# aniketntnu/WordDiffusion

Measured on AMD Instinct MI355X. Metric: denoised 64x256 word images/sec (1000-step DDPM), whole job, higher is better.
Workload: dtype bf16x3; 1 GPU; BASELINE configs[1]: batch 64 per GPU of 64x256 crops = [64,4,8,32] latents, 1000-step DDPM (999 executed steps), base unet.py UNetModel (320 ch, mult (1,1), 4 heads, 339 writers), random-init synthetic weights; variant=base, batch_per_gpu=64, noise_steps=1000, executed_steps_per_image=999, precision=split-bf16 MFMA x3, fp32 accumulate (<=1e-4 of the fp32 reference), output_finite=True

## Files before the change

### worddiffusion_amd/csrc/wd_gemm.hip

```cpp
#include <stdlib.h>

#include "wd_common.h"
#include "wd_gemm_epi.h"
#include "wd_gemm_priv.h"


namespace {

constexpr int BK = 32;

__device__ __forceinline__ int lds_off(int row, int ch) { return row * 64 + ((ch ^ ((row >> 2) & 3)) << 4); }
__device__ __forceinline__ int lds_off16(int row, int ch) { return row * 64 + ((ch ^ ((0 - (row >> 2)) & 3)) << 4); }


template <int BM, int BN, int TN, int NT>
__device__ __forceinline__ void wd_epilogue_lds(const wd_gemm_args& a, const f32x16 (&acc)[TN], char* smem, const int m0,
                                                const int n0, const int wm, const int wn, const int wcols, const int kh,
                                                const int nkh, const int tid, const int sidx = 0) {
    constexpr int LDE = BN + 4;
    float* ep = reinterpret_cast<float*>(smem);
    const int lane = tid & 63;
    const int frow = lane & 31, fhalf = lane >> 5;
    asm volatile("s_waitcnt vmcnt(0)" ::: "memory");
    __syncthreads();
// ... 2060 lines not shown
        if (!wd_epilogue_vec_ok(a)) return WD_EINVAL;
        if (a.tile == 0) a.tile = bm * 1000 + bn;
    }
    if (a.ksplit > 1 && (!a.ws || a.act == WD_ACT_GEGLU || a.w_layout == 1)) return WD_EINVAL;
    if (a.ln_gamma) {
        if (a.w_layout != 3 || (a.tile && a.tile != 64320) || a.n != 320 || a.ksplit > 1 || !a.ln_beta || !a.out_hi || (a.out_pl_ld & 3) ||
            ((reinterpret_cast<uintptr_t>(a.ln_gamma) | reinterpret_cast<uintptr_t>(a.ln_beta)) & 15) ||
            ((reinterpret_cast<uintptr_t>(a.out_hi) | reinterpret_cast<uintptr_t>(a.out_lo)) & 7) || a.act == WD_ACT_GEGLU)
            return WD_EINVAL;
        a.tile = 64320;
        a.ksplit = 1;
    }
    if (a.gn_gamma) {
        if (!a.gn_beta || !a.stat_part || !a.out_hi || (!a.ws && a.tile != 64080) || a.hw_out != 64 || a.m % 64 || a.n % 160 || a.gn_cpg <= 0 ||
            40 % a.gn_cpg || a.stat_cpg <= 0 || a.gn_cpg % a.stat_cpg || a.act != WD_ACT_NONE || a.resid_rows || a.w_layout == 1)
            return WD_EINVAL;
        if (!wd_epilogue_vec_ok(a) ||
            ((reinterpret_cast<uintptr_t>(a.ws) | reinterpret_cast<uintptr_t>(a.gn_gamma) | reinterpret_cast<uintptr_t>(a.gn_beta)) & 15))
            return WD_EINVAL;
        a.tickets = nullptr;
    }
    if (a.w_layout == 1) {
        a.ksplit = 1;
        a.tickets = nullptr;
    }
    if (a.nsrc < 1 || a.nsrc > 2 || (a.npass != 1 && a.npass != 3)) return WD_EINVAL;
    if (a.m <= 0 || a.n <= 0 || a.hw_out <= 0 || !a.w_hi || (a.npass == 3 && !a.w_lo)) return WD_EINVAL;
    if (!a.out_f32 && !a.out_hi) return WD_EINVAL;
    long k = 0;
    for (int s = 0; s < a.nsrc; ++s) {
        const wd_src& q = a.src[s];
        if (s == 0 && a.a32) {
            if (a.w_layout != 3 || a.npass != 3 || (a.tile && a.tile != 64320) || a.n % 320 || a.hw_out % 64 || !a.a32_part || !a.a32_gamma ||
                !a.a32_beta || a.a32_nchunk <= 0 || a.a32_pcpg <= 0 || a.a32_cpg <= 0 || a.a32_cpg % a.a32_pcpg || q.c % a.a32_cpg ||
                q.c > 1024 || a.a32_ld < q.c || (a.a32_ld & 3) || (reinterpret_cast<uintptr_t>(a.a32) & 15) || q.hw_src <= 0)
                return WD_EINVAL;
        } else if (!q.hi || (a.npass == 3 && !q.lo)) return WD_EINVAL;
        if (q.c <= 0 || q.c % BK || q.ld % 8 || q.ntaps < 1) return WD_EINVAL;
        if (!q.gather && q.ntaps != 1) return WD_EINVAL;
        if (q.gather && q.hw_src <= 0) return WD_EINVAL;
        k += (long)q.ntaps * q.c;
    }
    if (k != a.ktot) return WD_EINVAL;
    {
        const long lim = 0x7FFFFFF0L;
        if ((long)a.n * a.ktot * 2 >= lim) return WD_EINVAL;
        for (int s = 0; s < a.nsrc; ++s) {
            const wd_src& q = a.src[s];
            const long rows = q.gather ? (long)((a.m + a.hw_out - 1) / a.hw_out) * q.hw_src : (long)a.m;
            if ((s == 0 && a.a32) ? rows * a.a32_ld * 4 >= lim : rows * q.ld * 2 >= lim) return WD_EINVAL;
        }
    }
    if (a.act == WD_ACT_GEGLU && (a.n % 64 || a.tile == 0)) return WD_EINVAL;
    if (a.rowvec && a.rowvec_ld <= 0) return WD_EINVAL;
    if (a.resid && a.resid_ld <= 0) return WD_EINVAL;
    {
        const int nout = a.act == WD_ACT_GEGLU ? a.n / 2 : a.n;
        if ((a.out_f32 && a.out_ld < nout) || (a.out_hi && a.out_pl_ld < nout) || (a.resid && a.resid_ld < nout) ||
            (a.rowvec && a.rowvec_ld < nout))
            return WD_EINVAL;
        for (int s = 0; s < a.nsrc; ++s)
            if (!(s == 0 && a.a32) && a.src[s].ld < a.src[s].c) return WD_EINVAL;
    }

    if (a.w_layout == 3) {
        bool ok = a.src[0].ntaps <= 9 && (a.nsrc == 1 || (a.src[1].gather == nullptr && a.src[1].ntaps == 1));
        for (int s = 0; s < a.nsrc; ++s) ok = ok && (a.src[s].c % 64 == 0);
        if (!ok) return WD_EINVAL;
        const wd_src& q0 = a.src[0];
        const bool same3 = q0.ntaps == 9 && q0.gather && a.slab_rows > 0 && q0.hw_src == a.hw_out && a.hw_out % a.slab_rows == 0;
        const bool down3 = a.tile == 64080 && q0.ntaps == 9 && q0.gather && a.slab_rows > 0 && q0.hw_src == 4 * a.hw_out;
        if (!same3 && !down3) a.slab_rows = 0;
        a.tickets = nullptr;
        if (a.tile == 64080) {
            if (!wd_gemmq_applies(a)) return WD_EINVAL;
            if (a.gn_gamma && (40 % a.gn_cpg || 80 % a.gn_cpg)) return WD_EINVAL;
            r.a = a, r.kernel = K_GEMMQ;
            return WD_OK;
        }
        const int nk64 = a.ktot / 64;
        if (a.ksplit == 0) a.ksplit = a.ws ? wd_auto_ksplit(a.tile, a.m, a.n, nk64, a.ws_floats) : 1;
        if (a.ksplit > 1 && (nk64 < a.ksplit || (long)a.ksplit * a.m * a.n > a.ws_floats)) a.ksplit = 1;
        if (a.gn_gamma && a.ksplit <= 1) return WD_EINVAL;
        r.a = a, r.kernel = K_GEMMW;
        return WD_OK;
    }
#ifndef WDIFF_EXPERIMENTAL
    if (a.w_layout == 1) return WD_EINVAL;
#else
    if (a.w_layout == 1) {
        if (a.src[0].ntaps > 9 || a.slab_rows <= 0) return WD_EINVAL;
        if (a.nsrc == 2 && (a.src[1].gather || a.src[1].ntaps != 1)) return WD_EINVAL;
        if (a.tile == 0) a.tile = (a.act == WD_ACT_GEGLU || a.n % 160) ? 128064 : 128160;
        if (a.act == WD_ACT_GEGLU && a.n % (a.tile % 1000)) return WD_EINVAL;
        if (a.slab_rows > 192) return WD_EINVAL;
        if (a.tile != 128064 && a.tile != 128128 && a.tile != 128160) return WD_EINVAL;
        r.a = a, r.kernel = K_SLAB;
        return WD_OK;
    }
#endif
    bool conv3 = false;
    if (a.w_layout == 2) {
        const wd_src& q0 = a.src[0];
        static const int conv3_mode = getenv("WDIFF_CONV3") ? atoi(getenv("WDIFF_CONV3")) : 0;
#ifdef WDIFF_EXPERIMENTAL
        const bool conv3_env = conv3_mode != 0 || (a.dbg & 0x1000);
#else
        const bool conv3_env = false;
        (void)conv3_mode;
#endif
        const bool same3 = q0.ntaps == 9 && q0.gather && a.slab_rows > 0 && q0.hw_src == a.hw_out && a.hw_out % a.slab_rows == 0;
        conv3 = conv3_env && same3 && q0.c % 64 == 0 && a.act != WD_ACT_GEGLU && (a.tile == 0 || a.tile == 128160) &&
                (a.nsrc == 1 || (!a.src[1].gather && a.src[1].ntaps == 1 && a.src[1].c % 64 == 0));
        if (conv3) a.tile = 128160;
        a.w_layout = 0;
        static const bool arith_env = getenv("WDIFF_GEMM_ARITH_TAB") ? atoi(getenv("WDIFF_GEMM_ARITH_TAB")) != 0 : true;
        if (!same3 || !arith_env) a.slab_rows = 0;
    } else if (a.w_layout == 0) {
        a.slab_rows = 0;
    } else if (a.w_layout != 0) {
        return WD_EINVAL;
    }
    bool v2ok = (a.ktot % BK2 == 0) && !getenv("WDIFF_GEMM_V1");
    for (int s = 0; s < a.nsrc; ++s) v2ok = v2ok && (a.src[s].c % BK2 == 0);
    v2ok = v2ok && a.src[0].ntaps <= 9 && (a.nsrc == 1 || (a.src[1].gather == nullptr && a.src[1].ntaps == 1));
    const int nk64 = a.ktot / BK2;
    int tile = a.tile;
    if (tile == 0)
        tile = wd_auto_tile(a.m, a.n, nk64, v2ok && a.ws && a.ksplit == 0 && a.act != WD_ACT_GEGLU, a.ws_floats);
    if (a.ksplit == 0) {
        a.ksplit = (v2ok && a.ws && a.act != WD_ACT_GEGLU) ? wd_auto_ksplit(tile, a.m, a.n, nk64, a.ws_floats) : 1;
    }
    if (a.act == WD_ACT_GEGLU && a.n % (tile % 1000)) return WD_EINVAL;
    if (a.ksplit > 1 && (!v2ok || nk64 < a.ksplit || (long)a.ksplit * a.m * a.n > a.ws_floats)) a.ksplit = 1;
    bool use_v4 = false;
    if (tile == 128160) {
        static const int v4_env = getenv("WDIFF_GEMM_V4") ? atoi(getenv("WDIFF_GEMM_V4")) : 2;
        const long wgs = (long)((a.m + 127) / 128) * ((a.n + 159) / 160) * a.ksplit;
        use_v4 = v2ok && !a.stat_part && (v4_env == 1 || (v4_env == 2 && wgs >= 512) || (a.dbg & 0x400));
    }
    {
        static const bool fuse_env = getenv("WDIFF_GEMM_FUSE_COMBINE") ? atoi(getenv("WDIFF_GEMM_FUSE_COMBINE")) != 0 : false;
        const int bn = tile % 1000, bm = tile / 1000;
        const long ntile = (long)((a.m + bm - 1) / bm) * ((a.n + bn - 1) / bn);
        const bool aligned = (a.n & 3) == 0 && a.n % bn == 0 && wd_epilogue_vec_ok(a) && (reinterpret_cast<uintptr_t>(a.ws) & 15) == 0;
        if (!((fuse_env || (a.dbg & 0x2000)) && a.tickets && a.ksplit > 1 && v2ok && !use_v4 && !conv3 && aligned && ntile <= a.ntickets))
            a.tickets = nullptr;
    }
    if (a.gn_gamma && !(a.ksplit > 1 && tile == 128160 && v2ok && !use_v4 && !conv3)) return WD_EINVAL;
    static const int stagger_min = getenv("WDIFF_GEMM_STAGGER_MIN") ? atoi(getenv("WDIFF_GEMM_STAGGER_MIN")) : 10;
    static const bool stagger = getenv("WDIFF_GEMM_STAGGER") ? atoi(getenv("WDIFF_GEMM_STAGGER")) != 0 : true;
    static const bool m16 = getenv("WDIFF_GEMM_M16") ? atoi(getenv("WDIFF_GEMM_M16")) != 0 : true;
    static const bool pp = getenv("WDIFF_GEMM_PP") ? atoi(getenv("WDIFF_GEMM_PP")) != 0 : false;
    a.tile = tile;
#ifdef WDIFF_EXPERIMENTAL
    if (conv3 && v2ok) return r.a = a, r.kernel = K_CONV3, WD_OK;
#endif
    if (tile != 128064 && tile != 128160 && tile != 128128 && tile != 64064) return WD_EINVAL;
    if (tile == 128160) {
        if (use_v4) return r.a = a, r.kernel = K_V4, WD_OK;
#ifdef WDIFF_EXPERIMENTAL
        static const int v8_env = getenv("WDIFF_GEMM_V8") ? atoi(getenv("WDIFF_GEMM_V8")) : 0;
        bool v8ok = a.ktot % 32 == 0 && a.src[0].ntaps <= 9 && !a.stat_part && !a.gn_gamma && a.act != WD_ACT_GEGLU &&
                    (a.nsrc == 1 || (a.src[1].gather == nullptr && a.src[1].ntaps == 1));
        for (int s8 = 0; s8 < a.nsrc; ++s8) v8ok = v8ok && (a.src[s8].c % 32 == 0);
        if (v8ok && (v8_env == 1 || (a.dbg & 0x80000))) {
// ... 98 lines not shown
```

### worddiffusion_amd/csrc/wd_gemm_priv.h

```cpp
#pragma once
#include "wd_common.h"

int wd_gemmw_launch(const wd_gemm_args& a, hipStream_t st);
int wd_gemm_launch_reduce(const wd_gemm_args& a, hipStream_t st, int bm);
bool wd_gemmq_applies(const wd_gemm_args& a);
int wd_gemmq_launch(const wd_gemm_args& a, hipStream_t st);
```

### worddiffusion_amd/csrc/wd_gemmw.hip

```cpp
#include "wd_gemm_epi.h"
#include "wd_gemm_priv.h"

namespace {

constexpr int WNT = 512;

typedef __attribute__((ext_vector_type(4))) unsigned w_u32x4;

__device__ __forceinline__ int w_lds_off(int row, int ch) { return row * 128 + ((ch ^ ((row >> 1) & 7)) << 4); }

template <int NPASS, int RH, bool A32>
__global__ void __launch_bounds__(WNT, 1) wd_gemmw_kernel(const wd_gemm_args a, const int nbn, const int nbm) {
#if defined(__HIP_DEVICE_COMPILE__)
    constexpr int NPL = (NPASS == 1) ? 1 : 2;
    constexpr int BM = 64 * RH, BN = 320 / RH;
    constexpr int A_PL = BM * 128;
    constexpr int STAGE = NPL * A_PL;
    constexpr uint32_t WD_OOB = 0x80000000u;

    extern __shared__ __attribute__((aligned(16))) char smem[];
    int* s_tab = reinterpret_cast<int*>(smem + 2 * STAGE);

    const int ntile = nbn * nbm;
    const int nwg = ntile * a.ksplit;
    int wg;
    {
        const int bid = blockIdx.x;
        const int q = nwg >> 3, r = nwg & 7, xcd = bid & 7, loc = bid >> 3;
        wg = (xcd < r ? xcd * (q + 1) : r * (q + 1) + (xcd - r) * q) + loc;
    }
    const int sidx = wg % a.ksplit;
    wg /= a.ksplit;
    const int bn_i = wg % nbn, bm_i = wg / nbn;
    const int m0 = bm_i * BM, n0 = bn_i * BN;

    const int tid = threadIdx.x;
    const int lane = tid & 63;
    const int wave = __builtin_amdgcn_readfirstlane(tid >> 6);
    const int kh = wave >> 2;
    const int rh = RH == 2 ? (wave >> 1) & 1 : 0;
    const int cg = RH == 2 ? wave & 1 : wave & 3;
    const int l15 = lane & 15, lq = lane >> 4;

    {
        const int nt0 = a.src[0].ntaps;
        const int32_t* g0 = a.src[0].gather;
        const int hw_src0 = a.src[0].hw_src;
        const int Wimg = a.slab_rows;
        for (int idx = tid; idx < nt0 * BM; idx += WNT) {
            const int t = idx / BM, row = idx - t * BM;
            const int m = m0 + row;
            int v = -1;
            if (m < a.m) {
                if (g0 && Wimg > 0) {
                    const int b = m / a.hw_out, p = m - b * a.hw_out;
                    const int y = p / Wimg, x = p - y * Wimg;
                    const int ky = t / 3, dy = ky - 1, dx = t - ky * 3 - 1;
                    const int sy = y + dy, sx = x + dx;
                    if (sy >= 0 && sy * Wimg < a.hw_out && sx >= 0 && sx < Wimg) v = b * hw_src0 + sy * Wimg + sx;
                } else if (g0) {
                    const int b = m / a.hw_out, p = m - b * a.hw_out;
                    const int g = g0[t * a.hw_out + p];
                    if (g >= 0) v = b * hw_src0 + g;
                } else {
                    v = m;
                }
            }
            s_tab[idx] = v;
        }
    }
    float* s_aff = reinterpret_cast<float*>(s_tab + 9 * BM);
    if constexpr (A32) {
        const int c0 = a.src[0].c;
        const int b = m0 / a.hw_out;
        const int ngp = c0 / a.a32_pcpg, ratio = a.a32_cpg / a.a32_pcpg;
        for (int c = tid; c < c0; c += WNT) {
            const int g = c / a.a32_cpg;
            double su = 0.0, sq = 0.0;
            for (int k = 0; k < ratio; ++k)
                for (int ck = 0; ck < a.a32_nchunk; ++ck) {
                    const double* pp = a.a32_part + (((long)b * a.a32_nchunk + ck) * ngp + g * ratio + k) * 2;
                    su += pp[0];
                    sq += pp[1];
                }
            const double n = (double)a.src[0].hw_src * a.a32_cpg;
            const double mu = su / n;
            double var = sq / n - mu * mu;
            if (var < 0.0) var = 0.0;
            const float rstd = (float)(1.0 / sqrt(var + (double)a.a32_eps));
            const float sc = rstd * a.a32_gamma[c];
            s_aff[2 * c] = sc;
            s_aff[2 * c + 1] = a.a32_beta[c] - (float)mu * sc;
        }
    }
    __syncthreads();
    unsigned long long skipmask = 0;
    if (RH == 1 && a.src[0].gather) {
        for (int t = 0; t < a.src[0].ntaps; ++t) {
            const unsigned long long oob = __ballot(s_tab[t * BM + lane] < 0);
#pragma unroll
            for (int i = 0; i < 4; ++i)
                if (((oob >> (16 * i)) & 0xFFFFull) == 0xFFFFull) skipmask |= 1ull << (4 * t + i);
        }
    }

    auto make_srd = [](const wd_bf16* p) {
        return __builtin_amdgcn_make_buffer_rsrc(const_cast<wd_bf16*>(p), 0, 0x7FFFFFF0, 0x00020000);
    };
    const int nct = a.n >> 4;
    const long wgrp = a.w_ngroups > 1 ? (long)((m0 % a.hw_out) / (a.hw_out / a.w_ngroups)) * a.w_group_stride : 0;
    const __amdgpu_buffer_rsrc_t srd_w_hi = make_srd(a.w_hi + wgrp), srd_w_lo = make_srd((a.w_lo ? a.w_lo : a.w_hi) + wgrp);
    const uint32_t b_voff = (uint32_t)(((n0 >> 4) + 5 * cg) * 1024 + lane * 16);
    const uint32_t kstep_bytes = (uint32_t)nct * 1024u;

    const int arow = tid >> 3, ach = tid & 7;
    const int a_dst = w_lds_off(arow, ach);

    const int nk_all = a.ktot / 64;
    const int k_begin = __builtin_amdgcn_readfirstlane((int)((long)nk_all * sidx / a.ksplit));
    const int k_end = __builtin_amdgcn_readfirstlane((int)((long)nk_all * (sidx + 1) / a.ksplit));
    const int nk = k_end - k_begin;
    const int cpt0 = a.src[0].c >> 6, n0st = a.src[0].ntaps * cpt0;
    int s = 0, tap = 0, kc = 0, left;
    int cur_ld = a.src[0].ld, cur_cpt = cpt0;
    if (k_begin < n0st) {
        tap = __builtin_amdgcn_readfirstlane(k_begin / cpt0);
        kc = k_begin - tap * cpt0;
        left = n0st - k_begin;
    } else {
        s = 1;
        kc = k_begin - n0st;
        cur_ld = a.src[1].ld;
        cur_cpt = a.src[1].c >> 6;
        left = cur_cpt - kc;
    }
    const __amdgpu_buffer_rsrc_t srd0_hi = make_srd(A32 ? reinterpret_cast<const wd_bf16*>(a.a32) : a.src[0].hi),
                                 srd0_lo = make_srd(A32 ? reinterpret_cast<const wd_bf16*>(a.a32) : (a.src[0].lo ? a.src[0].lo : a.src[0].hi));
    const wd_bf16* p1h = a.nsrc > 1 ? a.src[1].hi : a.src[0].hi;
    const wd_bf16* p1l = a.nsrc > 1 ? (a.src[1].lo ? a.src[1].lo : a.src[1].hi) : p1h;
    const __amdgpu_buffer_rsrc_t srd1_hi = make_srd(p1h), srd1_lo = make_srd(p1l);
    uint32_t a_voff[RH];
    auto locate = [&]() {
        int ln;
        asm volatile("v_mbcnt_lo_u32_b32 %0, -1, 0\n\tv_mbcnt_hi_u32_b32 %0, -1, %0" : "=v"(ln));
#pragma unroll
        for (int j = 0; j < RH; ++j) {
            const int row = wave * 8 + (ln >> 3) + 64 * j;
            int r;
            if (s == 0) r = s_tab[tap * BM + row];
            else r = (m0 + row < a.m) ? m0 + row : -1;
            if (A32 && s == 0) a_voff[j] = r >= 0 ? (uint32_t)r * (uint32_t)(a.a32_ld * 4) + (uint32_t)(ach * 32) : WD_OOB;
            else a_voff[j] = r >= 0 ? (uint32_t)r * (uint32_t)(cur_ld * 2) + (uint32_t)(ach * 16) : WD_OOB;
        }
    };
    locate();
    auto kabs = [&]() { return s == 0 ? tap * cpt0 + kc : n0st + kc; };
    auto advance = [&]() {
        --left;
        const bool sw1 = left == 0 && (s + 1 < a.nsrc);
        ++kc;
        bool relocate = false;
        if (kc == cur_cpt) {
            kc = 0;
            ++tap;
            relocate = true;
        }
        if (sw1) {
            s = 1;
            tap = 0;
            kc = 0;
            cur_ld = a.src[1].ld;
            cur_cpt = a.src[1].c >> 6;
            left = cur_cpt;
            relocate = true;
        }
        if (relocate) locate();
    };
    int kb = 0;

    w_u32x4 ra[RH][NPL];
    int ra_ch = 0;
    bool ra_ok[RH];
    auto load_a = [&](const bool live) {
        if (A32) ra_ch = (s == 0) ? kc * 64 + ach * 8 : -1;
#pragma unroll
        for (int j = 0; j < RH; ++j) {
            const uint32_t vo = live ? a_voff[j] : WD_OOB;
            if (A32) ra_ok[j] = vo != WD_OOB;
            if (A32 && s == 0) {
                static_assert(!A32 || NPL == 2, "the fp32 source path holds eight floats in the two plane registers");
                ra[j][0] = __builtin_amdgcn_raw_buffer_load_b128(srd0_hi, vo, kc * 256, 0);
                ra[j][NPL - 1] = __builtin_amdgcn_raw_buffer_load_b128(srd0_hi, vo + 16, kc * 256, 0);
            } else {
#pragma unroll
                for (int p = 0; p < NPL; ++p) {
                    if (s == 0) ra[j][p] = __builtin_amdgcn_raw_buffer_load_b128(p ? srd0_lo : srd0_hi, vo, kc * 128, 0);
                    else ra[j][p] = __builtin_amdgcn_raw_buffer_load_b128(p ? srd1_lo : srd1_hi, vo, kc * 128, 0);
                }
            }
        }
    };
    auto store_a = [&](char* base) {
        if (A32 && ra_ch >= 0) {
            const float4* tab = reinterpret_cast<const float4*>(s_aff + 2 * ra_ch);
            const float4 t0 = tab[0], t1 = tab[1], t2 = tab[2], t3 = tab[3];
            const bool silu = a.a32_silu != 0;
#pragma unroll
            for (int j = 0; j < RH; ++j) {
                const float4 x0 = __builtin_bit_cast(float4, ra[j][0]), x1 = __builtin_bit_cast(float4, ra[j][NPL - 1]);
                float4 y0, y1;
                y0.x = x0.x * t0.x + t0.y; y0.y = x0.y * t0.z + t0.w; y0.z = x0.z * t1.x + t1.y; y0.w = x0.w * t1.z + t1.w;
                y1.x = x1.x * t2.x + t2.y; y1.y = x1.y * t2.z + t2.w; y1.z = x1.z * t3.x + t3.y; y1.w = x1.w * t3.z + t3.w;
                if (silu) {
                    y0.x = wd_silu(y0.x); y0.y = wd_silu(y0.y); y0.z = wd_silu(y0.z); y0.w = wd_silu(y0.w);
                    y1.x = wd_silu(y1.x); y1.y = wd_silu(y1.y); y1.z = wd_silu(y1.z); y1.w = wd_silu(y1.w);
                }
                if (!ra_ok[j]) y0 = y1 = make_float4(0.f, 0.f, 0.f, 0.f);
                uint2 h0, l0, h1, l1;
                wd_split4(y0, h0, l0);
                wd_split4(y1, h1, l1);
                *reinterpret_cast<w_u32x4*>(base + j * 8192 + a_dst) = w_u32x4{h0.x, h0.y, h1.x, h1.y};
                *reinterpret_cast<w_u32x4*>(base + (NPL - 1) * A_PL + j * 8192 + a_dst) = w_u32x4{l0.x, l0.y, l1.x, l1.y};
            }
        } else {
#pragma unroll
            for (int j = 0; j < RH; ++j)
#pragma unroll
                for (int p = 0; p < NPL; ++p) *reinterpret_cast<w_u32x4*>(base + p * A_PL + j * 8192 + a_dst) = ra[j][p];
        }
    };
    auto load_b = [&](bf16x8 (&fb)[5][NPL], const bool live) {
        const uint32_t so = live ? (uint32_t)(2 * kb + kh) * kstep_bytes : 0u;
        const uint32_t vo = live ? b_voff : WD_OOB;
#pragma unroll
        for (int t = 0; t < 5; ++t)
#pragma unroll
            for (int p = 0; p < NPL; ++p)
                fb[t][p] = __builtin_bit_cast(bf16x8, __builtin_amdgcn_raw_buffer_load_b128(p ? srd_w_lo : srd_w_hi, vo + t * 1024, so, 0));
    };

    f32x4 acc[4][5];
#pragma unroll
    for (int i = 0; i < 4; ++i)
#pragma unroll
        for (int t = 0; t < 5; ++t)
#pragma unroll
            for (int r = 0; r < 4; ++r) acc[i][t][r] = 0.0f;

    bf16x8 xb[5][NPL], yb[5][NPL];
    bf16x8 xa[4][NPL];
    auto read_a = [&](const char* base) {
        const int ch = kh * 4 + lq;
#pragma unroll
        for (int i = 0; i < 4; ++i) {
            const int ao = w_lds_off(rh * 64 + i * 16 + l15, ch);
#pragma unroll
            for (int p = 0; p < NPL; ++p) xa[i][p] = *reinterpret_cast<const bf16x8*>(base + p * A_PL + ao);
        }
    };
    auto mfma_all = [&](const bf16x8 (&fb)[5][NPL], const int skip) {
        if constexpr (RH == 1) {
#pragma unroll
            for (int i = 0; i < 4; ++i) {
                if (skip & (1 << i)) continue;
#pragma unroll
                for (int t = 0; t < 5; ++t) {
                    if (NPL == 2) {
                        acc[i][t] = __builtin_amdgcn_mfma_f32_16x16x32_bf16(xa[i][NPL - 1], fb[t][0], acc[i][t], 0, 0, 0);
                        acc[i][t] = __builtin_amdgcn_mfma_f32_16x16x32_bf16(xa[i][0], fb[t][NPL - 1], acc[i][t], 0, 0, 0);
                    }
                    acc[i][t] = __builtin_amdgcn_mfma_f32_16x16x32_bf16(xa[i][0], fb[t][0], acc[i][t], 0, 0, 0);
                }
            }
        } else {
#pragma unroll
            for (int t = 0; t < 5; ++t) {
#pragma unroll
                for (int i = 0; i < 4; ++i) {
                    if (NPL == 2) {
                        acc[i][t] = __builtin_amdgcn_mfma_f32_16x16x32_bf16(xa[i][NPL - 1], fb[t][0], acc[i][t], 0, 0, 0);
                        acc[i][t] = __builtin_amdgcn_mfma_f32_16x16x32_bf16(xa[i][0], fb[t][NPL - 1], acc[i][t], 0, 0, 0);
                    }
                    acc[i][t] = __builtin_amdgcn_mfma_f32_16x16x32_bf16(xa[i][0], fb[t][0], acc[i][t], 0, 0, 0);
                }
            }
        }
    };
    const uint32_t cpt0_inv = (65536u + (uint32_t)cpt0 - 1u) / (uint32_t)cpt0;
    auto skip_of = [&](const int kit) {
        if constexpr (RH != 1) return 0;
        const int ka = k_begin + kit;
        const int tp = (int)(((uint32_t)ka * cpt0_inv) >> 16);
        int sk = (ka < n0st && ka < 1024) ? (int)((skipmask >> (4 * tp)) & 15ull) : 0;
        if (kit >= nk) sk = 15;
        return __builtin_amdgcn_readfirstlane(sk);
    };

    kb = kabs();
    load_a(nk > 0);
    if (nk > 0) advance();
    load_b(xb, nk > 0);
    store_a(smem);
    kb = kabs();
    load_a(nk > 1);
    if (nk > 1) advance();
#ifdef WD_GEMMW_STAMPS
    const bool stamp = (a.dbg & 0x100) && blockIdx.x == 0 && lane == 0 && a.ws;
    unsigned long long* sb = reinterpret_cast<unsigned long long*>(a.ws) + (long)wave * ((nk + 1) & ~1) * 4;
#define WD_STAMP(i) if (stamp) sb[kit * 4 + (i)] = __builtin_amdgcn_s_memtime()
#define WD_STAMP_LGKM() if (stamp) asm volatile("s_waitcnt lgkmcnt(0)" ::: "memory")
#else
#define WD_STAMP(i)
#define WD_STAMP_LGKM()
#endif
    if (kh == 0 || (a.dbg & 0x4000)) {
        auto half_step = [&](const int kit, const bf16x8 (&bcur)[5][NPL], bf16x8 (&bnext)[5][NPL]) {
            __builtin_amdgcn_sched_barrier(0);
            WD_STAMP(0);
            __syncthreads();
            WD_STAMP(1);
            const char* base = smem + (kit & 1) * STAGE;
            char* nbase = smem + ((kit + 1) & 1) * STAGE;
            store_a(nbase);
            load_b(bnext, kit + 1 < nk);
            kb = kabs();
            load_a(kit + 2 < nk);
            if (kit + 2 < nk) advance();
            read_a(base);
            __builtin_amdgcn_sched_barrier(0);
            WD_STAMP_LGKM();
            WD_STAMP(2);
            mfma_all(bcur, skip_of(kit));
            __builtin_amdgcn_sched_barrier(0);
            WD_STAMP(3);
        };
        for (int kit = 0; kit < nk; kit += 2) {
            half_step(kit, xb, yb);
            half_step(kit + 1, yb, xb);
        }
    } else {
        auto late_step = [&](const int kit, bf16x8 (&bset)[5][NPL]) {
            __builtin_amdgcn_sched_barrier(0);
            WD_STAMP(0);
            __syncthreads();
            WD_STAMP(1);
            const char* base = smem + (kit & 1) * STAGE;
            char* nbase = smem + ((kit + 1) & 1) * STAGE;
            if (kit > 0) mfma_all(bset, skip_of(kit - 1));
            __builtin_amdgcn_sched_barrier(0);
            WD_STAMP(2);
            store_a(nbase);
            load_b(bset, kit + 1 < nk);
            kb = kabs();
            load_a(kit + 2 < nk);
            if (kit + 2 < nk) advance();
            read_a(base);
            __builtin_amdgcn_sched_barrier(0);
            WD_STAMP_LGKM();
            WD_STAMP(3);
        };
        for (int kit = 0; kit < nk; kit += 2) {
            late_step(kit, yb);
            late_step(kit + 1, xb);
        }
        if (nk > 0) mfma_all(yb, skip_of(((nk + 1) & ~1) - 1));
    }
#undef WD_STAMP
#undef WD_STAMP_LGKM

    constexpr int LDE = BN + 4;
    float* ep = reinterpret_cast<float*>(smem);
    __syncthreads();
    for (int hh = 0; hh < 2; ++hh) {
        if (kh == hh) {
#pragma unroll
            for (int i = 0; i < 4; ++i)
#pragma unroll
                for (int t = 0; t < 5; ++t)
#pragma unroll
                    for (int r = 0; r < 4; ++r) {
                        float* pe = ep + (rh * 64 + i * 16 + 4 * lq + r) * LDE + cg * 80 + t * 16 + l15;
                        *pe = (hh == 0) ? acc[i][t][r] : *pe + acc[i][t][r];
                    }
        }
        __syncthreads();
    }
    wd_epilogue_tail<BM, BN, WNT>(a, ep, m0, n0, tid, sidx);
#endif
}

__global__ void __launch_bounds__(256) wd_pack_w_kernel(const wd_bf16* __restrict__ hi, const wd_bf16* __restrict__ lo, const int n,
                                                        const int ktot, wd_bf16* __restrict__ out_hi, wd_bf16* __restrict__ out_lo) {
    const long i = (long)blockIdx.x * 256 + threadIdx.x;
    const long total = (long)n * ktot / 8;
    if (i >= total) return;
    const int nct = n >> 4;
    const int l = (int)(i & 63);
    const long blk = i >> 6;
    const int ct = (int)(blk % nct);
    const long ks = blk / nct;
    const long src = (long)(ct * 16 + (l & 15)) * ktot + ks * 32 + (l >> 4) * 8;
    reinterpret_cast<uint4*>(out_hi)[i] = *reinterpret_cast<const uint4*>(hi + src);
    if (lo) reinterpret_cast<uint4*>(out_lo)[i] = *reinterpret_cast<const uint4*>(lo + src);
}

template <int NPASS, int RH, bool A32 = false>
int launchw(const wd_gemm_args& a, hipStream_t st) {
    constexpr int NPL = (NPASS == 1) ? 1 : 2;
    constexpr int BM = 64 * RH, BN = 320 / RH;
    constexpr int loop_smem = 2 * NPL * BM * 128 + 9 * BM * 4 + (A32 ? 2 * 1024 * 4 : 0);
    constexpr int red_smem = BM * (BN + 4) * 4 + WD_STAT_SCRATCH;
    constexpr int smem = loop_smem > red_smem ? loop_smem : red_smem;
    static bool attr_done = false;
    if (!attr_done) {
        if (hipFuncSetAttribute(reinterpret_cast<const void*>(&wd_gemmw_kernel<NPASS, RH, A32>), hipFuncAttributeMaxDynamicSharedMemorySize,
                                smem) != hipSuccess)
            return WD_ELAUNCH;
        attr_done = true;
    }
    const int nbn = a.n / BN, nbm = (a.m + BM - 1) / BM;
    {
        WdLaunchScope scope(WD_CLS_GEMM_WDIRECT, st, 2.0 * (double)a.m * (double)a.n * (double)a.ktot);
        hipLaunchKernelGGL((wd_gemmw_kernel<NPASS, RH, A32>), dim3(nbn * nbm * a.ksplit), dim3(WNT), smem, st, a, nbn, nbm);
    }
    if (a.ksplit > 1) return wd_gemm_launch_reduce(a, st, BM);
    return wd_check_launch();
}

}

int wd_gemmw_launch(const wd_gemm_args& a, hipStream_t st) {
    if (a.a32) return launchw<3, 1, true>(a, st);
    if (a.tile == 128160) return a.npass == 3 ? launchw<3, 2>(a, st) : launchw<1, 2>(a, st);
    return a.npass == 3 ? launchw<3, 1>(a, st) : launchw<1, 1>(a, st);
}

extern "C" int wd_gemm_pack_w(const wd_bf16* hi, const wd_bf16* lo, int n, int ktot, wd_bf16* out_hi, wd_bf16* out_lo, void* stream) {
    if (!hi || !out_hi || (lo && !out_lo) || n <= 0 || ktot <= 0 || n % 16 || ktot % 32) return WD_EINVAL;
    const long total = (long)n * ktot / 8;
    hipStream_t st = reinterpret_cast<hipStream_t>(stream);
    WdLaunchScope scope(WD_CLS_OTHER, st);
    hipLaunchKernelGGL(wd_pack_w_kernel, dim3((unsigned)((total + 255) / 256)), dim3(256), 0, st, hi, lo, n, ktot, out_hi, out_lo);
    return wd_check_launch();
}
```

### worddiffusion_amd/engine.py

```python
from __future__ import annotations

import ctypes as C
import math
import os
from typing import Dict, List, Optional, Tuple

import numpy as np
import torch

from . import _native as N
from .layers import (DownsampleParams, ResBlockParams, SpatialTransformerParams, UpsampleParams)


def conv_gather_table(h: int, w: int, mode: str) -> Tuple[np.ndarray, int, int]:
    if mode == "same":
        ho, wo = h, w
    elif mode == "down":
        ho, wo = (h + 2 - 3) // 2 + 1, (w + 2 - 3) // 2 + 1
    elif mode == "up":
        ho, wo = 2 * h, 2 * w
    elif mode == "down_rb":
        ho, wo = (h - 2) // 2 + 1, (w - 2) // 2 + 1
    else:
        raise ValueError(mode)
# ... 197 lines not shown
                    hi, lo, ld, ntc = d.data_ptr() + 4 * col_off, 0, 0, 1
                    nch = (n + vchunk - 1) // vchunk
                else:
                    ld = r.cols
                    o = 2 * (row_off * ld + col_off)
                    hi, lo = d[0].data_ptr() + o, d[1].data_ptr() + o
                    ntc = (c + tile - 1) // tile
                    nch = (((npad if mode == 1 else n) + tile - 1) // tile) * ntc
                recs.append(N.WdRepackEntry(p.data_ptr(), p2.data_ptr() if p2 is not None else 0, hi, lo, n, c, t,
                                            mode, npad, ld, g, ntc, c0, 0, 0))
                c0 += nch
                if frag is not None and name in frag and self.frag_ok(r):
                    f = frag[name]
                    recs.append(N.WdRepackEntry(p.data_ptr(), 0, f[0].data_ptr(), f[1].data_ptr(), n, c, t, 3, 0,
                                                r.rows, g, ntc, c0, row_off, col_off))
                    c0 += nch
        raw = torch.frombuffer((N.WdRepackEntry * len(recs))(*recs), dtype=torch.uint8).to(dev)
        return raw, c0, len(recs)


class Act:
    __slots__ = ("t", "c", "h", "w", "stats", "prod", "perm")

    def __init__(self, t, c, h, w, stats=None, prod=None, perm=None):
        self.t, self.c, self.h, self.w = t, c, h, w
        self.perm = perm
        self.stats = stats
        self.prod = prod


class Plan:
    def __init__(self):
        self.cond: List[tuple] = []
        self.step: List[tuple] = []
        self.keep: List[object] = []
        self.out: Optional[torch.Tensor] = None

    @staticmethod
    def _run(ops, stream):
        for fn, args, what in ops:
            rc = fn(*args, stream)
            if rc != 0:
                N.check(rc, what)

    def run_cond(self, stream):
        self._run(self.cond, stream)

    def run_film(self, stream):
        self._run(getattr(self, "film", []), stream)
        self.film_loaded = -1

    @staticmethod
    def film_prepare(t, stream):
        return False

    def run_step(self, stream):
        self._run(self.step, stream)

    def run_step1(self, stream):
        self._run(self.step1, stream)


def _ptr(t: Optional[torch.Tensor], byte_off: int = 0):
    return None if t is None else t.data_ptr() + byte_off


class UNetEngine:

    fold_proj = False

    def __init__(self, model, variant: str):
        self.model = model
        self.variant = variant
        self.lib = N.lib()
        self.npass = 3
        self._sig = None
        self._ps, self._ps_gen = None, -1
        self._pack = None
        self._w: Dict[str, torch.Tensor] = {}
        self._w3: Dict[str, torch.Tensor] = {}
        self._w3_meta: Dict[str, tuple] = {}
        self._wf: Dict[str, torch.Tensor] = {}
        self.use_wdirect = os.environ.get("WDIFF_GEMM_WDIRECT", "1") != "0"
        self.use_up_phases = os.environ.get("WDIFF_UPSAMPLE_PHASES", "1") != "0"
        self._derived: Dict[str, tuple] = {}
        self.use_smallmap = os.environ.get("WDIFF_GEMM_SMALLMAP", "1") != "0"
        self.fuse_ff = os.environ.get("WDIFF_FUSE_FF", "1") != "0"
        self.fuse_proj = os.environ.get("WDIFF_FUSE_PROJ", "1") != "0"
        self.fuse_ln = os.environ.get("WDIFF_FUSE_LN", "1") != "0"
        self.fuse_gn_in = int(os.environ.get("WDIFF_FUSE_GN_IN", "1"))
        self.use_slab = os.environ.get("WDIFF_SLAB", "0") != "0"
        self.fuse_stats = os.environ.get("WDIFF_FUSE_STATS", "1") != "0"
        self.fuse_xattn = os.environ.get("WDIFF_FUSE_XATTN", "1") != "0"
        self.use_conv3 = os.environ.get("WDIFF_CONV3", "0") != "0"
        if (self.use_slab or self.use_conv3) and not self.lib.wd_gemm_experimental():
            raise N.NativeError("WDIFF_SLAB / WDIFF_CONV3 need a library built with WDIFF_EXPERIMENTAL=1 "
                                "(python -m worddiffusion_amd.build --force)")
        self.fuse_xattn_pair = os.environ.get("WDIFF_FUSE_XATTN_PAIR", "1") != "0"
        self.fuse_st = os.environ.get("WDIFF_FUSE_ST", "1") != "0"
        self.fold_proj = os.environ.get("WDIFF_FOLD_PROJ", "1") != "0"
        self.fuse_out = os.environ.get("WDIFF_FUSE_OUT", "1") != "0"
        self.fuse_in = os.environ.get("WDIFF_FUSE_IN", "1") != "0"
        self.pack_kv = os.environ.get("WDIFF_PACK_KV", "1") != "0"
        self.fuse_gn2 = os.environ.get("WDIFF_FUSE_GN2", "1") != "0"
        self.fuse_gn = os.environ.get("WDIFF_FUSE_GN", "1") != "0"
        self.fuse_split = os.environ.get("WDIFF_FUSE_SPLIT", "1") != "0"
        self._plans: Dict[tuple, Plan] = {}
        self._tabs: Dict[tuple, torch.Tensor] = {}
        self._tab_np: Dict[int, np.ndarray] = {}
        self._same_w: Dict[int, int] = {}
        self._down_w: Dict[int, int] = {}
        self._ws = None
        self.device = None

    def set_precision(self, mode: str):
        npass = {"bf16x3": 3, "fp32": 3, "bf16": 1}[mode]
        if npass != self.npass:
            self.npass = npass
            self._plans.clear()

    def _recipes(self) -> "RecipeBook":
        m = self.model
        R = RecipeBook()
        film_w = []
        self.film_off = {}
        off = 0
        cin_conv = m.input_blocks[0][0]
        self.kpad_in = ((9 * cin_conv.in_channels + 31) // 32) * 32
        R.matrix("in.w", cin_conv.out_channels, self.kpad_in).fwd(cin_conv.weight)
        R.vector("in.b", cin_conv.bias)
        R.vector("in.w.f32", cin_conv.weight)
        R.linear("te0", m.time_embed[0])
        R.linear("te2", m.time_embed[2])
        if m.num_classes is not None:
            R.vector("label", m.label_emb.weight)
        we = m.word_emb
        cd = we.embedding.weight.shape[1]
        R.vector("we.table", we.embedding.weight)
        qkv = (we.attention.linear_query, we.attention.linear_key, we.attention.linear_value)
        R.matrix("we.qkv.w", 3 * cd, cd)
        R.vector_cat("we.qkv.b", [l.bias for l in qkv])
        for i, l in enumerate(qkv):
            R["we.qkv.w"].fwd(l.weight, row_off=i * cd)
        kv_w = []
        self.kv_off = {}
        kvo = 0
        for name, mod in self._walk():
            if isinstance(mod, ResBlockParams):
                R.vector(name + ".gn1.g", mod.in_layers[0].weight)
                R.vector(name + ".gn1.b", mod.in_layers[0].bias)
                R.matrix(name + ".c1.w", mod.cout, 9 * mod.cin).fwd(mod.in_layers[2].weight)
                R.vector(name + ".c1.b", mod.in_layers[2].bias)
                R.vector(name + ".gn2.g", mod.out_layers[0].weight)
                R.vector(name + ".gn2.b", mod.out_layers[0].bias)
                if mod.cin != mod.cout:
                    R.matrix(name + ".c2.w", mod.cout, 9 * mod.cout + mod.cin).fwd(mod.out_layers[3].weight) \
                        .fwd(mod.skip_connection.weight, col_off=9 * mod.cout)
                    R.vector(name + ".c2.b", mod.out_layers[3].bias, mod.skip_connection.bias)
                else:
                    R.matrix(name + ".c2.w", mod.cout, 9 * mod.cout).fwd(mod.out_layers[3].weight)
                    R.vector(name + ".c2.b", mod.out_layers[3].bias)
                film_w.append(mod.emb_layers[1])
                self.film_off[name] = off
                off += mod.cout
            elif isinstance(mod, (DownsampleParams, UpsampleParams)):
                conv = mod.op if isinstance(mod, DownsampleParams) else mod.conv
# ... 173 lines not shown
            self._tab_np[dt.data_ptr()] = tab
            if mode == "down":
                self._down_w[dt.data_ptr()] = wo
            if mode == "same":
                self._same_w[dt.data_ptr()] = w
        return self._tabs[key]

    def _f32(self, P: Plan, *shape):
        t = torch.empty(shape, dtype=torch.float32, device=self.device)
        P.keep.append(t)
        return t

    def _planes(self, P: Plan, rows, ld):
        t = torch.zeros((2, rows, ld), dtype=torch.bfloat16, device=self.device)
        P.keep.append(t)
        return t

    def _hilo(self, planes: Optional[torch.Tensor], byte_off: int = 0):
        if planes is None:
            return None, None
        return planes[0].data_ptr() + byte_off, (planes[1].data_ptr() + byte_off if self.npass == 3 else None)

    def _src(self, planes: torch.Tensor, c: int, ntaps: int = 1, gather: Optional[torch.Tensor] = None,
             hw_src: int = 0, col_off: int = 0) -> N.WdSrc:
        s = N.WdSrc()
        s._tab_np = self._tab_np.get(gather.data_ptr()) if gather is not None else None
        s._same_w = self._same_w.get(gather.data_ptr(), 0) if gather is not None else 0
        s._down_w = self._down_w.get(gather.data_ptr(), 0) if gather is not None else 0
        ld = planes.shape[2]
        s.hi = planes[0].data_ptr() + 2 * col_off
        s.lo = planes[1].data_ptr() + 2 * col_off
        s.gather = _ptr(gather)
        s.ld, s.c, s.ntaps, s.hw_src = ld, c, ntaps, hw_src
        return s

    def _gemm(self, ops, what, srcs, wname, m, hw_out, bias=None, rowvec=None, rowvec_ld=0, resid=None,
              resid_ld=0, resid_rows=None, act=N.ACT_NONE, out_f32=None, out_ld=0, out_pl=None, n=None, tile=0,
              w_row_off=0, want_stats=False, a32=None, ln=None, w_groups=None):
        a = N.WdGemmArgs()
        for i, s in enumerate(srcs):
            a.src[i] = s
        a.nsrc = len(srcs)
        a.npass = self.npass
        wp = self._w[wname]
        ktot = wp.shape[2]
        assert ktot == sum(s.ntaps * s.c for s in srcs), (what, ktot, [(s.ntaps, s.c) for s in srcs])
        nrows = wp.shape[1] if n is None else n
        a.w_hi = wp[0].data_ptr() + 2 * w_row_off * ktot
        a.w_lo = wp[1].data_ptr() + 2 * w_row_off * ktot
        a.m, a.n, a.ktot, a.hw_out = m, nrows, ktot, hw_out
        a.bias = _ptr(bias)
        a.rowvec, a.rowvec_ld = rowvec, rowvec_ld
        a.resid, a.resid_ld, a.resid_rows = resid, resid_ld, resid_rows
        a.act = act
        a.out_f32, a.out_ld = _ptr(out_f32), out_ld
        if out_pl is not None:
            a.out_hi, a.out_lo, a.out_pl_ld = out_pl[0].data_ptr(), out_pl[1].data_ptr(), out_pl.shape[2]
        if a32 is not None:
            self._set_a32(a, *a32)
        if w_groups is not None:
            a.w_ngroups, a.w_group_stride = w_groups
        a.tile = tile
        if self._ws is None:
            self._ws = torch.empty(128 * 128 * 160 * 8, dtype=torch.float32, device=self.device)
        a.ksplit, a.ws, a.ws_floats = 0, self._ws.data_ptr(), self._ws.numel()
        self._give_tickets(a, m, nrows)
        span = 0
        if self.use_slab and w_row_off == 0 and (len(srcs) == 1 or (srcs[1].ntaps == 1 and not srcs[1].gather)):
            tabnp = getattr(srcs[0], "_tab_np", None)
            span = slab_span(tabnp, hw_out, srcs[0].hw_src, m)
            if span > 192 or ((m + 127) // 128) * max(1, nrows // 160) < 96:
                span = 0
        s0 = srcs[0]
        frag = not span and not self.use_conv3 and w_row_off == 0 and n is None and act == N.ACT_NONE and tile == 0
        width = (getattr(s0, "_down_w", 0) or getattr(s0, "_same_w", 0)) if s0.ntaps == 9 else 0
        wdirect = (frag and self.use_wdirect and wdirect_fills_chip(m, nrows) and
                   self._legal(a, w_layout=3, tile=64320, slab_rows=getattr(s0, "_same_w", 0) if s0.ntaps == 9 else 0))
        smallmap = (frag and not wdirect and self.use_smallmap and hw_out == 64 and 128 <= (m // 64) * (nrows // 80) <= 512 and
                    self._legal(a, w_layout=3, tile=64080, slab_rows=width))
        assert (a32 is None and w_groups is None) or wdirect, what
        if wdirect or smallmap:
            wf = self._wfrag(wname)
            a.w_hi, a.w_lo = wf[0].data_ptr(), wf[1].data_ptr()
        elif span:
            meta = (srcs[0].ntaps, srcs[0].c, srcs[1].c if len(srcs) > 1 else 0)
            if wname not in self._w3:
                self._w3[wname] = slab_order(wp, *meta)
                self._w3_meta[wname] = meta
            assert self._w3_meta[wname] == meta, wname
            w3 = self._w3[wname]
            a.w_hi, a.w_lo = w3[0].data_ptr(), w3[1].data_ptr()
            a.w_layout, a.slab_rows = 1, span
        else:
            same_w = getattr(srcs[0], "_same_w", 0)
            if (same_w and srcs[0].ntaps == 9 and srcs[0].c % 64 == 0 and act == N.ACT_NONE and tile == 0 and
                    (len(srcs) == 1 or (srcs[1].ntaps == 1 and not srcs[1].gather and srcs[1].c % 64 == 0))):
                a.w_layout, a.slab_rows = 2, same_w
        a._ln_pl = None
        if ln is not None and self.fuse_ln and not self.use_slab:
            pl = torch.zeros((2, m, nrows), dtype=torch.bfloat16, device=self.device)
            if self._legal(a, out_hi=pl[0].data_ptr(), out_lo=pl[1].data_ptr(), out_pl_ld=nrows, ln_gamma=self._w[ln + ".g"].data_ptr(),
                           ln_beta=self._w[ln + ".b"].data_ptr(), ln_eps=1e-5):
                self._cur_plan.keep.append(pl)
                a._ln_pl = pl
        stats = None
        if want_stats and self.fuse_stats and nrows % 32 == 0 and (hw_out % 128 == 0 or hw_out == 64) and not span:
            cpg = nrows // 32
            r = self._resolved(a, stat_part=a.ws, stat_cpg=cpg)
            if r is not None:
                nchunk = max(1, hw_out // (r.tile // 1000))
                part = torch.zeros((m // hw_out, nchunk, 32, 2), dtype=torch.float64, device=self.device)
                self._cur_plan.keep.append(part)
                a.stat_part, a.stat_cpg = part.data_ptr(), cpg
                stats = (part, nchunk, cpg)
        a._stats = stats
        self._cur_plan.keep.append(a)
        ops.append((self.lib.wd_gemm, (C.byref(a),), what))
        return a

    def _resolved(self, a, **fields) -> Optional[N.WdGemmArgs]:
        b = N.WdGemmArgs.from_buffer_copy(a)
        for k, v in fields.items():
            setattr(b, k, v)
        out = N.WdGemmArgs()
        return out if self.lib.wd_gemm_check(C.byref(b), C.byref(out)) == N.WD_OK else None

    def _legal(self, a, apply=True, **fields) -> bool:
        if self._resolved(a, **fields) is None:
            return False
        if apply:
            for k, v in fields.items():
                setattr(a, k, v)
        return True

    def _set_a32(self, a, x32: "Act", gname, eps, silu):
        part, nchunk, pc = x32.stats
        a.a32, a.a32_ld, a.a32_part = x32.t.data_ptr(), x32.c, part.data_ptr()
        a.a32_nchunk, a.a32_pcpg, a.a32_cpg = nchunk, pc, x32.c // 32
        a.a32_gamma, a.a32_beta = self._w[gname + ".g"].data_ptr(), self._w[gname + ".b"].data_ptr()
        a.a32_eps, a.a32_silu = float(eps), int(silu)

    def _wdirect_ok(self, srcs, m, n, hw_out, a32=None, **fields) -> bool:
        a = N.WdGemmArgs()
        for i, s in enumerate(srcs):
            a.src[i] = s
        a.nsrc, a.npass, a.m, a.n, a.ktot, a.hw_out = len(srcs), self.npass, m, n, sum(s.ntaps * s.c for s in srcs), hw_out
        a.w_layout, a.tile = 3, 64320
        a.w_hi = a.w_lo = a.out_f32 = 16
        a.out_ld = n
        if a32 is not None:
            self._set_a32(a, *a32)
        return self._legal(a, apply=False, **fields)

    def _give_tickets(self, a, m, n):
        ntick = ((m + 63) // 64) * ((n + 63) // 64)
        if ntick > 2048:
            return
        P = self._cur_plan
        tk = getattr(P, "_tickets", None)
        if tk is None or P._ticket_off + ntick > tk.numel():
            tk = torch.zeros(1 << 16, dtype=torch.int32, device=self.device)
            P.keep.append(tk)
            P._tickets, P._ticket_off = tk, 0
        a.tickets, a.ntickets = tk.data_ptr() + 4 * P._ticket_off, ntick
        P._ticket_off += ntick

# ... 764 lines not shown
```

Baseline: 36.55 images/s.

## Add slab-staged A operand path to wdirect 3x3 conv GEMM kernel

Adds a SLAB variant of the wdirect 64x320 split-bf16 GEMM kernel. For same-resolution 3x3 convs it loads a halo'd activation slab (rows plus borders) per channel chunk into LDS once and reuses it across all 9 taps by shifting LDS offsets. This replaces per-tap gathered A loads. The aim is to cut global/L2 traffic and gather-table overhead. It costs more LDS, a different sync pattern, and skips k-split, and it is enabled by default when the shape fits.

Result: faster. 37.55 images/s (median of 6 runs) (+2.7%).

```diff
diff --git a/worddiffusion_amd/csrc/wd_gemm.hip b/worddiffusion_amd/csrc/wd_gemm.hip
--- a/worddiffusion_amd/csrc/wd_gemm.hip
+++ b/worddiffusion_amd/csrc/wd_gemm.hip
@@ -2166,6 +2166,15 @@
         if (a.ksplit == 0) a.ksplit = a.ws ? wd_auto_ksplit(a.tile, a.m, a.n, nk64, a.ws_floats) : 1;
         if (a.ksplit > 1 && (nk64 < a.ksplit || (long)a.ksplit * a.m * a.n > a.ws_floats)) a.ksplit = 1;
         if (a.gn_gamma && a.ksplit <= 1) return WD_EINVAL;
+        {
+            static const bool slab_env = getenv("WDIFF_GEMMW_SLAB") ? atoi(getenv("WDIFF_GEMMW_SLAB")) != 0 : WD_GEMMW_SLAB_DEFAULT;
+            const bool want = (a.dbg & WD_GEMMW_SLAB_OFF) ? false : (a.dbg & WD_GEMMW_SLAB_ON) ? true : slab_env;
+            const bool fits = a.tile == 64320 && a.npass == 3 && a.ksplit <= 1 && a.w_ngroups <= 1 && !a.a32 && !a.ln_gamma && same3 &&
+                              64 % a.slab_rows == 0 && a.hw_out % 64 == 0 && a.m % a.hw_out == 0 && q0.c % 64 == 0 &&
+                              (a.nsrc == 1 || (a.src[1].gather == nullptr && a.src[1].ntaps == 1));
+            a.dbg &= ~(WD_GEMMW_SLAB_OFF | WD_GEMMW_SLAB_ON);
+            if (want && fits) a.dbg |= WD_GEMMW_SLAB_BIT;
+        }
         r.a = a, r.kernel = K_GEMMW;
         return WD_OK;
     }
diff --git a/worddiffusion_amd/csrc/wd_gemm_priv.h b/worddiffusion_amd/csrc/wd_gemm_priv.h
--- a/worddiffusion_amd/csrc/wd_gemm_priv.h
+++ b/worddiffusion_amd/csrc/wd_gemm_priv.h
@@ -2,6 +2,8 @@
 #include "wd_common.h"
 
 int wd_gemmw_launch(const wd_gemm_args& a, hipStream_t st);
+constexpr bool WD_GEMMW_SLAB_DEFAULT = true;
+constexpr int WD_GEMMW_SLAB_OFF = 0x8000, WD_GEMMW_SLAB_ON = 0x10000, WD_GEMMW_SLAB_BIT = WD_GEMMW_SLAB_ON;
 int wd_gemm_launch_reduce(const wd_gemm_args& a, hipStream_t st, int bm);
 bool wd_gemmq_applies(const wd_gemm_args& a);
 int wd_gemmq_launch(const wd_gemm_args& a, hipStream_t st);
diff --git a/worddiffusion_amd/csrc/wd_gemmw.hip b/worddiffusion_amd/csrc/wd_gemmw.hip
--- a/worddiffusion_amd/csrc/wd_gemmw.hip
+++ b/worddiffusion_amd/csrc/wd_gemmw.hip
@@ -9,9 +9,10 @@
 
 __device__ __forceinline__ int w_lds_off(int row, int ch) { return row * 128 + ((ch ^ ((row >> 1) & 7)) << 4); }
 
-template <int NPASS, int RH, bool A32>
+template <int NPASS, int RH, bool A32, bool SLAB = false>
 __global__ void __launch_bounds__(WNT, 1) wd_gemmw_kernel(const wd_gemm_args a, const int nbn, const int nbm) {
 #if defined(__HIP_DEVICE_COMPILE__)
+    static_assert(!SLAB || (NPASS == 3 && RH == 1 && !A32), "the slab form is the split-bf16 64 x 320 kernel over operand planes");
     constexpr int NPL = (NPASS == 1) ? 1 : 2;
     constexpr int BM = 64 * RH, BN = 320 / RH;
     constexpr int A_PL = BM * 128;
@@ -19,6 +20,9 @@
     constexpr uint32_t WD_OOB = 0x80000000u;
 
     extern __shared__ __attribute__((aligned(16))) char smem[];
+    const int Wm = SLAB ? a.slab_rows : 1, wsh = __builtin_ctz(Wm);
+    const int TR = 64 >> wsh, NR = TR + 2, SW = Wm + 2;
+    const int CPL = NR * SW * 128, CHB = 2 * CPL;
     int* s_tab = reinterpret_cast<int*>(smem + 2 * STAGE);
 
     const int ntile = nbn * nbm;
@@ -42,7 +46,7 @@
     const int cg = RH == 2 ? wave & 1 : wave & 3;
     const int l15 = lane & 15, lq = lane >> 4;
 
-    {
+    if constexpr (!SLAB) {
         const int nt0 = a.src[0].ntaps;
         const int32_t* g0 = a.src[0].gather;
         const int hw_src0 = a.src[0].hw_src;
@@ -95,7 +99,7 @@
     }
     __syncthreads();
     unsigned long long skipmask = 0;
-    if (RH == 1 && a.src[0].gather) {
+    if (!SLAB && RH == 1 && a.src[0].gather) {
         for (int t = 0; t < a.src[0].ntaps; ++t) {
             const unsigned long long oob = __ballot(s_tab[t * BM + lane] < 0);
 #pragma unroll
@@ -117,10 +121,10 @@
     const int a_dst = w_lds_off(arow, ach);
 
     const int nk_all = a.ktot / 64;
+    const int cpt0 = a.src[0].c >> 6, n0st = a.src[0].ntaps * cpt0;
     const int k_begin = __builtin_amdgcn_readfirstlane((int)((long)nk_all * sidx / a.ksplit));
     const int k_end = __builtin_amdgcn_readfirstlane((int)((long)nk_all * (sidx + 1) / a.ksplit));
-    const int nk = k_end - k_begin;
-    const int cpt0 = a.src[0].c >> 6, n0st = a.src[0].ntaps * cpt0;
+    const int nk = SLAB ? 0 : k_end - k_begin;
     int s = 0, tap = 0, kc = 0, left;
     int cur_ld = a.src[0].ld, cur_cpt = cpt0;
     if (k_begin < n0st) {
@@ -153,7 +157,7 @@
             else a_voff[j] = r >= 0 ? (uint32_t)r * (uint32_t)(cur_ld * 2) + (uint32_t)(ach * 16) : WD_OOB;
         }
     };
-    locate();
+    if constexpr (!SLAB) locate();
     auto kabs = [&]() { return s == 0 ? tap * cpt0 + kc : n0st + kc; };
     auto advance = [&]() {
         --left;
@@ -296,14 +300,152 @@
         return __builtin_amdgcn_readfirstlane(sk);
     };
 
-    kb = kabs();
-    load_a(nk > 0);
-    if (nk > 0) advance();
-    load_b(xb, nk > 0);
-    store_a(smem);
-    kb = kabs();
-    load_a(nk > 1);
-    if (nk > 1) advance();
+    if constexpr (SLAB) {
+        const wd_src& q0 = a.src[0];
+        const int H = a.hw_out >> wsh;
+        const int bsm = m0 / a.hw_out;
+        const int y0 = (m0 - bsm * a.hw_out) >> wsh;
+        const int ntok = NR * Wm;
+        const int cpt1 = a.nsrc > 1 ? a.src[1].c >> 6 : 0, nch = cpt0 + cpt1;
+        const int nst = 9 * cpt0 + cpt1;
+        int skm0 = 0, skm2 = 0;
+        int ub[4];
+#pragma unroll
+        for (int i = 0; i < 4; ++i) {
+            if (y0 + ((16 * i + 15) >> wsh) < 1) skm0 |= 1 << i;
+            if (y0 + ((16 * i) >> wsh) + 1 >= H) skm2 |= 1 << i;
+            ub[i] = ((16 * i) >> wsh) * SW + ((16 * i) & (Wm - 1));
+        }
+        const uint32_t frow_bytes = (uint32_t)(q0.ld * 2), frow1_bytes = (uint32_t)(a.src[1].ld * 2);
+        int fdst = -1;
+        auto slab_piece = [&](const int t, const int chunk, const bool live) -> uint32_t {
+            int ln;
+            asm volatile("v_mbcnt_lo_u32_b32 %0, -1, 0\n\tv_mbcnt_hi_u32_b32 %0, -1, %0" : "=v"(ln));
+            const int tq = wave * 8 + (ln >> 3) + 64 * t, fpc = ln & 7;
+            if (chunk >= cpt0) {
+                const bool piece = live && tq < 64;
+                fdst = piece ? w_lds_off(tq, fpc) : -1;
+                return piece ? (uint32_t)(m0 + tq) * frow1_bytes + (uint32_t)(fpc * 16) : WD_OOB;
+            }
+            const int fy = tq >> wsh, fx = tq & (Wm - 1);
+            const int gy = y0 - 1 + fy;
+            const bool piece = live && tq < ntok;
+            fdst = piece ? w_lds_off(fy * SW + fx + 1, fpc) : -1;
+            return (piece && gy >= 0 && gy < H) ? (uint32_t)(bsm * q0.hw_src + gy * Wm + fx) * frow_bytes + (uint32_t)(fpc * 16) : WD_OOB;
+        };
+        auto slab_load = [&](const int t, const int chunk, const bool live) {
+            const uint32_t vo = slab_piece(t, chunk, live);
+            if (chunk < cpt0) {
+                ra[0][0] = __builtin_amdgcn_raw_buffer_load_b128(srd0_hi, vo, chunk * 128, 0);
+                ra[0][1] = __builtin_amdgcn_raw_buffer_load_b128(srd0_lo, vo, chunk * 128, 0);
+            } else {
+                ra[0][0] = __builtin_amdgcn_raw_buffer_load_b128(srd1_hi, vo, (chunk - cpt0) * 128, 0);
+                ra[0][1] = __builtin_amdgcn_raw_buffer_load_b128(srd1_lo, vo, (chunk - cpt0) * 128, 0);
+            }
+        };
+        auto slab_store = [&](char* buf, const int t, const int chunk, const bool live) {
+            slab_piece(t, chunk, live);
+            if (fdst >= 0) {
+                *reinterpret_cast<w_u32x4*>(buf + fdst) = ra[0][0];
+                *reinterpret_cast<w_u32x4*>(buf + CPL + fdst) = ra[0][1];
+            }
+        };
+        for (int i = tid; i < 2 * 2 * NR * 2 * 8; i += WNT) {
+            const int pc = i & 7, side = (i >> 3) & 1;
+            int rest = i >> 4;
+            const int ry = rest % NR;
+            rest /= NR;
+            const int pl = rest & 1, bf = rest >> 1;
+            *reinterpret_cast<w_u32x4*>(smem + bf * CHB + pl * CPL + w_lds_off(ry * SW + (side ? SW - 1 : 0), pc)) = w_u32x4{0u, 0u, 0u, 0u};
+        }
+        kb = 0;
+        load_b(xb, true);
+        {
+            w_u32x4 v[3][2];
+#pragma unroll
+            for (int t = 0; t < 3; ++t) {
+                slab_load(t, 0, true);
+                v[t][0] = ra[0][0], v[t][1] = ra[0][1];
+            }
+#pragma unroll
+            for (int t = 0; t < 3; ++t) {
+                ra[0][0] = v[t][0], ra[0][1] = v[t][1];
+                slab_store(smem, t, 0, true);
+            }
+        }
+        int st = 0, sc = 0;
+        int pft = 0, pfc = -1;
+        auto mem_phase = [&](const int kit, bf16x8 (&bnext)[5][NPL]) {
+            const bool conv = sc < cpt0;
+            if (pfc >= 0) slab_store(smem + (pfc & 1) * CHB, pft, pfc, true);
+            int tn = st + 1, cn = sc;
+            if (tn == (conv ? 9 : 1)) tn = 0, cn = sc + 1;
+            kb = cn < cpt0 ? tn * cpt0 + cn : n0st + cn - cpt0;
+            load_b(bnext, kit + 1 < nst);
+            const bool two = !conv || (st == 8 && sc == cpt0 - 1);
+            const int fc = two ? sc + 2 : sc + 1, ft = two ? 0 : st;
+            const bool freal = fc < nch && 64 * ft < (fc < cpt0 ? ntok : 64);
+            pfc = freal ? fc : -1, pft = ft;
+            if (freal) slab_load(ft, fc, true);
+            const int ky = (st * 11) >> 5;
+            const int shift = ky * SW + (st - 3 * ky);
+            const char* cb = smem + (sc & 1) * CHB;
+            int ln;
+            asm volatile("v_mbcnt_lo_u32_b32 %0, -1, 0\n\tv_mbcnt_hi_u32_b32 %0, -1, %0" : "=v"(ln));
+            const int f15 = ln & 15, ch = kh * 4 + (ln >> 4);
+            const int frow = conv ? shift + (f15 >> wsh) * SW + (f15 & (Wm - 1)) : f15;
+#pragma unroll
+            for (int i = 0; i < 4; ++i) {
+                const int ao = w_lds_off((conv ? ub[i] : 16 * i) + frow, ch);
+#pragma unroll
+                for (int p = 0; p < NPL; ++p) xa[i][p] = *reinterpret_cast<const bf16x8*>(cb + p * CPL + ao);
+            }
+            int sk = !conv ? 0 : ky == 0 ? skm0 : ky == 2 ? skm2 : 0;
+            if (kit >= nst) sk = 15;
+            st = tn, sc = cn;
+            return __builtin_amdgcn_readfirstlane(sk);
+        };
+        if (kh == 0) {
+            auto early_step = [&](const int kit, const bf16x8 (&bcur)[5][NPL], bf16x8 (&bnext)[5][NPL]) {
+                __builtin_amdgcn_sched_barrier(0);
+                if (st == 0 || kit == 1) __syncthreads();
+                const int sk = mem_phase(kit, bnext);
+                __builtin_amdgcn_sched_barrier(0);
+                mfma_all(bcur, sk);
+                __builtin_amdgcn_sched_barrier(0);
+            };
+            for (int kit = 0; kit < nst; kit += 2) {
+                early_step(kit, xb, yb);
+                early_step(kit + 1, yb, xb);
+            }
+        } else {
+            int psk = 15;
+            auto late_step = [&](const int kit, bf16x8 (&bset)[5][NPL]) {
+                __builtin_amdgcn_sched_barrier(0);
+                if (st == 0 || kit == 1) __syncthreads();
+                mfma_all(bset, psk);
+                __builtin_amdgcn_sched_barrier(0);
+                psk = mem_phase(kit, bset);
+                __builtin_amdgcn_sched_barrier(0);
+            };
+            for (int kit = 0; kit < nst; kit += 2) {
+                late_step(kit, yb);
+                late_step(kit + 1, xb);
+            }
+            mfma_all(yb, psk);
+        }
+    }
+
+    if constexpr (!SLAB) {
+        kb = kabs();
+        load_a(nk > 0);
+        if (nk > 0) advance();
+        load_b(xb, nk > 0);
+        store_a(smem);
+        kb = kabs();
+        load_a(nk > 1);
+        if (nk > 1) advance();
+    }
 #ifdef WD_GEMMW_STAMPS
     const bool stamp = (a.dbg & 0x100) && blockIdx.x == 0 && lane == 0 && a.ws;
     unsigned long long* sb = reinterpret_cast<unsigned long long*>(a.ws) + (long)wave * ((nk + 1) & ~1) * 4;
@@ -427,9 +569,33 @@
     return wd_check_launch();
 }
 
+int launchw_slab(const wd_gemm_args& a, hipStream_t st) {
+    constexpr int red_smem = 64 * (320 + 4) * 4 + WD_STAT_SCRATCH;
+    constexpr int max_loop = 2 * 2 * 198 * 128;
+    constexpr int max_smem = max_loop > red_smem ? max_loop : red_smem;
+    static_assert(max_smem <= 160 * 1024, "LDS budget");
+    const int W = a.slab_rows;
+    const int loop_smem = 2 * 2 * (64 / W + 2) * (W + 2) * 128;
+    const int smem = loop_smem > red_smem ? loop_smem : red_smem;
+    static bool attr_done = false;
+    if (!attr_done) {
+        if (hipFuncSetAttribute(reinterpret_cast<const void*>(&wd_gemmw_kernel<3, 1, false, true>), hipFuncAttributeMaxDynamicSharedMemorySize,
+                                max_smem) != hipSuccess)
+            return WD_ELAUNCH;
+        attr_done = true;
+    }
+    const int nbn = a.n / 320, nbm = a.m / 64;
+    {
+        WdLaunchScope scope(WD_CLS_GEMM_WDIRECT, st, 2.0 * (double)a.m * (double)a.n * (double)a.ktot);
+        hipLaunchKernelGGL((wd_gemmw_kernel<3, 1, false, true>), dim3(nbn * nbm), dim3(WNT), smem, st, a, nbn, nbm);
+    }
+    return wd_check_launch();
 }
 
+}
+
 int wd_gemmw_launch(const wd_gemm_args& a, hipStream_t st) {
+    if (a.dbg & WD_GEMMW_SLAB_BIT) return launchw_slab(a, st);
     if (a.a32) return launchw<3, 1, true>(a, st);
     if (a.tile == 128160) return a.npass == 3 ? launchw<3, 2>(a, st) : launchw<1, 2>(a, st);
     return a.npass == 3 ? launchw<3, 1>(a, st) : launchw<1, 1>(a, st);
diff --git a/worddiffusion_amd/engine.py b/worddiffusion_amd/engine.py
--- a/worddiffusion_amd/engine.py
+++ b/worddiffusion_amd/engine.py
@@ -303,6 +303,7 @@
         self._w3_meta: Dict[str, tuple] = {}
         self._wf: Dict[str, torch.Tensor] = {}
         self.use_wdirect = os.environ.get("WDIFF_GEMM_WDIRECT", "1") != "0"
+        self.gemmw_slab = {None: None, "0": False}.get(os.environ.get("WDIFF_GEMMW_SLAB"), True)
         self.use_up_phases = os.environ.get("WDIFF_UPSAMPLE_PHASES", "1") != "0"
         self._derived: Dict[str, tuple] = {}
         self.use_smallmap = os.environ.get("WDIFF_GEMM_SMALLMAP", "1") != "0"
@@ -642,6 +643,8 @@
         if wdirect or smallmap:
             wf = self._wfrag(wname)
             a.w_hi, a.w_lo = wf[0].data_ptr(), wf[1].data_ptr()
+            if wdirect and self.gemmw_slab is not None:
+                a.dbg |= 0x10000 if self.gemmw_slab else 0x8000
         elif span:
             meta = (srcs[0].ntaps, srcs[0].c, srcs[1].c if len(srcs) > 1 else 0)
             if wname not in self._w3:
```
